# ruanyyyyyyy/point-cloud-process

Hardware: AMD Instinct MI355X
Metric: correspondence-pairs/sec + ms/ICP-iter, 120k-pt KITTI pair (higher is better)
Workload: dtype f64; 1 GPU; point-to-point ICP iteration, 120000 x 120000 KITTI-shaped synthetic scan pair per GPU (BASELINE configs[1]); exact 1-NN via grid; nn=grid, pairs_per_gpu=1, points_src=120000, points_tgt=120000

## Files before the change

point-cloud-process_amd/csrc/pcr_grid_search.hip:

```cpp
#include <atomic>
#include <chrono>
#include <cmath>
#include <cstdlib>
#include <cstring>
#include "pcr_descent.h"
#include "pcr_icp_step.h"

constexpr unsigned int HARD_SCAN_T = 192;
constexpr int HARD_STACK = 160;
constexpr long long ID_NONE = 0x7fffffffffffffffll;
constexpr int H_NLIST = 32;
constexpr int H_CSTRIDE = 32;
__host__ __device__ static inline unsigned int hard_list_cap(long long nq) {
    const long long halves = (nq + 15) / 16;
    return (unsigned int)(((halves + H_NLIST - 1) / H_NLIST) * 16 + 64);
}

template <int G>
__device__ static inline void group_best(double& bd2, long long& bid, unsigned int& bpos) {
#pragma unroll
    for (int off = G / 2; off > 0; off >>= 1) {
        const double od2 = __shfl_xor(bd2, off, 64);
        const long long oid = __shfl_xor(bid, off, 64);
        const unsigned int opos = __shfl_xor(bpos, off, 64);
// ... 649 lines not shown
        const cell_entry en = L->stack[sp];
        const double ecell = gv.cell0 * (double)(1ll << (2 * en.level));
        if (box_dist2(gv, en.level, ecell, en.x, en.y, en.z, ax, ay, az) > bound2) continue;
        const int cl = en.level - 1;
        const unsigned int CX = en.x * 4u + (lane & 3), CY = en.y * 4u + ((lane >> 2) & 3), CZ = en.z * 4u + (lane >> 4);
        const double cdist = box_dist2(gv, cl, ecell * 0.25, CX, CY, CZ, ax, ay, az);
        unsigned int cs = 0, ce = 0;
        const bool cvalid = cdist <= bound2 && lookup_cell(gv.table[cl], gv.mask[cl], CX, CY, CZ, &cs, &ce);
        hard_disperse(gv, L, sp, lane, cvalid, cs, ce, CX, CY, CZ, cl, cdist, ax, ay, az, bd2, bid, bpos, bound2, n_pts, bw);
        ++h_steps;
    }
}

__device__ __forceinline__ static void hard_search(const pcr_grid_view& gv, hard_lds* L, const int lane, const double ax, const double ay, const double az,
                                                   double bound2, bool have_cand, double& bd2, long long& bid, unsigned int& bpos,
                                                   unsigned int& h_steps, unsigned int& h_pts, int& s_level0, double* win = nullptr) {
    double bw[3] = {0.0, 0.0, 0.0};
    const int top = gv.levels - 1;
    bd2 = DBL_MAX;
    bid = ID_NONE;
    bpos = POS_NONE;
    bool clamped = false;
    const int cx = cell_coord(ax, gv.lo[0], gv.inv_cell0, &clamped);
    const int cy = cell_coord(ay, gv.lo[1], gv.inv_cell0, &clamped);
    const int cz = cell_coord(az, gv.lo[2], gv.inv_cell0, &clamped);
    if (!clamped && !have_cand) {
        unsigned int s, e;
        if (lookup_cell(gv.table[0], gv.mask[0], (unsigned int)cx, (unsigned int)cy, (unsigned int)cz, &s, &e)) {
            scan_range(gv.pts, s + lane, e, 64, ax, ay, az, bd2, bid, bpos, bw);
            bound2 = fmin(bound2, wave_min_f64(bd2));
        }
    }
    auto level_for = [&](double b2, int from) {
        double c = gv.cell0 * (double)(1ll << (2 * from));
        for (int l = from; l <= top; ++l) {
            const double safe = c * (1.0 - 1e-9);
            if (safe * safe >= b2) return l;
            c *= 4.0;
        }
        return top + 1;
    };
    have_cand = have_cand || __any(bd2 < DBL_MAX);
    int s_level = clamped ? top + 1 : (have_cand ? level_for(bound2, 0) : 0);
    s_level0 = s_level;
    int sp = 0;
    while (s_level <= top) {
        const int lvl = s_level;
        const double cell = gv.cell0 * (double)(1ll << (2 * lvl));
        bool valid = lane < 27;
        const int X = (cx >> (2 * lvl)) + (lane % 3 - 1), Y = (cy >> (2 * lvl)) + ((lane / 3) % 3 - 1), Z = (cz >> (2 * lvl)) + (lane / 9 - 1);
        const int lim = (int)(PCR_COORD_MAX >> (2 * lvl));
        valid = valid && X >= 0 && Y >= 0 && Z >= 0 && X <= lim && Y <= lim && Z <= lim;
        unsigned int s = 0, e = 0;
        double bdist = 0.0;
        if (valid) {
            bdist = box_dist2(gv, lvl, cell, (unsigned int)X, (unsigned int)Y, (unsigned int)Z, ax, ay, az);
            valid = bdist <= bound2 && lookup_cell(gv.table[lvl], gv.mask[lvl], (unsigned int)X, (unsigned int)Y, (unsigned int)Z, &s, &e);
        }
        hard_disperse(gv, L, sp, lane, valid, s, e, (unsigned int)X, (unsigned int)Y, (unsigned int)Z, lvl, bdist, ax, ay, az, bd2, bid, bpos,
                      bound2, h_pts, bw);
        ++h_steps;
        hard_drain(gv, L, sp, lane, ax, ay, az, bd2, bid, bpos, bound2, h_steps, h_pts, bw);
        const double safe = cell * (1.0 - 1e-9);
        if (safe * safe >= bound2) break;
        s_level = (bound2 < DBL_MAX) ? level_for(bound2, lvl + 1) : lvl + 1;
    }
    if (s_level > top) {
        const double cell = gv.cell0 * (double)(1ll << (2 * top));
        const int b0 = (int)(PCR_COORD_BIAS >> (2 * top));
        bool valid = lane < 8;
        const unsigned int X = b0 + (lane & 1), Y = b0 + ((lane >> 1) & 1), Z = b0 + ((lane >> 2) & 1);
        unsigned int s = 0, e = 0;
        double bdist = 0.0;
        if (valid) {
            bdist = box_dist2(gv, top, cell, X, Y, Z, ax, ay, az);
            valid = bdist <= bound2 && lookup_cell(gv.table[top], gv.mask[top], X, Y, Z, &s, &e);
        }
        hard_disperse(gv, L, sp, lane, valid, s, e, X, Y, Z, top, bdist, ax, ay, az, bd2, bid, bpos, bound2, h_pts, bw);
        ++h_steps;
        hard_drain(gv, L, sp, lane, ax, ay, az, bd2, bid, bpos, bound2, h_steps, h_pts, bw);
    }
    {
        const double m = wave_min_f64(bd2);
        unsigned long long cm = __ballot(bpos != POS_NONE && bd2 == m);
        if (!cm) { bd2 = DBL_MAX; bid = ID_NONE; bpos = POS_NONE; if (win) { win[0] = win[1] = win[2] = 0.0; } return; }
        int wl = (int)__ffsll((long long)cm) - 1;
        cm &= cm - 1;
        if (cm) {
            long long best_id = readlane_i64(bid, wl);
            while (cm) {
                const int l = (int)__ffsll((long long)cm) - 1;
                cm &= cm - 1;
                const long long id_l = readlane_i64(bid, l);
                if (id_l < best_id) { best_id = id_l; wl = l; }
            }
        }
        bd2 = m;
        bid = readlane_i64(bid, wl);
        bpos = (unsigned int)__builtin_amdgcn_readlane((int)bpos, wl);
        if (win) {
#pragma unroll
            for (int k = 0; k < 3; ++k)
                win[k] = readlane_f64(bw[k], wl);
        }
    }
}

__global__ void __launch_bounds__(256)
grid_hard_kernel(pcr_grid_view gv, const work_item* __restrict__ list, const unsigned int* __restrict__ count_p, long long nq, double max_d2, int gated,
                 unsigned int* __restrict__ res_pos, double* __restrict__ res_d2, unsigned long long* __restrict__ dbg,
                 const pcr_icp_dev_state* __restrict__ st) {
    __shared__ hard_lds s_lds[4];
    if (st && st->stop) return;
    const int lane = threadIdx.x & 63, wave = threadIdx.x >> 6;
    hard_lds* L = &s_lds[wave];
    unsigned int l_cnt = lane < H_NLIST ? count_p[H_CSTRIDE * lane] : 0u;
    unsigned int l_inc = l_cnt;
#pragma unroll
    for (int off = 1; off < H_NLIST; off <<= 1) {
        const unsigned int o = __shfl_up(l_inc, off, 64);
        if (lane >= off) l_inc += o;
    }
    const unsigned int count = __shfl(l_inc, H_NLIST - 1, 64);
    const unsigned int l_exc = l_inc - l_cnt;
    const unsigned int l_cap = hard_list_cap(nq);
    for (unsigned int w = blockIdx.x * 4 + wave; w < count; w += gridDim.x * 4) {
        const int hl = (int)__ffsll((long long)__ballot(lane < H_NLIST && l_exc <= w && w < l_exc + l_cnt)) - 1;
        const work_item it = list[(size_t)hl * l_cap + (w - __shfl(l_exc, hl, 64))];
        const unsigned long long h_t0 = dbg ? __builtin_amdgcn_s_memtime() : 0;
        unsigned int h_steps = 0, h_pts = 0;
        int s_level0 = 0;
        double bd2;
        long long bid;
        unsigned int bpos;
        hard_search(gv, L, lane, it.ax, it.ay, it.az, gated ? fmin(it.best_d2, max_d2) : it.best_d2, it.best_pos != POS_NONE, bd2, bid, bpos, h_steps,
                    h_pts, s_level0);
        if (lane == 0) {
            res_pos[it.qi] = bpos;
            if (res_d2) res_d2[it.qi] = bd2;
            if (dbg && w < 60000) {
                dbg[(1 << 17) + w * 4 + 0] = __builtin_amdgcn_s_memtime() - h_t0;
                dbg[(1 << 17) + w * 4 + 1] = ((unsigned long long)h_steps << 32);
                dbg[(1 << 17) + w * 4 + 2] = h_pts;
                dbg[(1 << 17) + w * 4 + 3] = (unsigned long long)(it.best_pos != POS_NONE) | ((unsigned long long)(s_level0 + 1) << 8);
            }
        }
    }
}

constexpr int ACC_SETS = 32;
constexpr int PASS_GROUPS = 32;
constexpr int PASS_SYNC_STRIDE = 32;
constexpr int PASS_SYNC_WORDS = PASS_SYNC_STRIDE * (PASS_GROUPS + 1);
constexpr unsigned long long ITEM_NONE = ~0ull;
constexpr unsigned int POISON_HI = 0xfffffffeu;
__device__ static inline unsigned long long item_poison(unsigned int pass_id) { return ((unsigned long long)POISON_HI << 32) | pass_id; }
#ifndef PCR_PASS_SPIN_LIMIT
#define PCR_PASS_SPIN_LIMIT (1u << 21)
#endif
constexpr unsigned int PASS_SPIN_LIMIT = PCR_PASS_SPIN_LIMIT;
constexpr int Q_BITS = 22;
constexpr unsigned long long Q_MASK = (1ull << Q_BITS) - 1ull;
constexpr long long PASS_MAX_NQ = 1ll << 26;
struct pass_args {
    unsigned long long* items;
    unsigned long long* sync;
    unsigned int cap;
    unsigned long long* acc;
    wt_xyz* prev_xyz;
    double scale, inv_scale;
    pcr_icp_dev_state* st;
    pcr_icp_loop_args la;
    unsigned int* tile_cost;
    unsigned int pass_id;
    unsigned long long* host_block;
    unsigned int notify;
    unsigned int* plog;
};
constexpr int PASS_LOG_WORDS = 3 * PCR_ICP_MAX_LOG + 8;
constexpr size_t HOST_LOG_OFF = (sizeof(pcr_icp_dev_state) + 63) & ~(size_t)63;
constexpr size_t HOST_FLAG_OFF = 8192 - 8;
static_assert(HOST_LOG_OFF + 4 * PASS_LOG_WORDS <= HOST_FLAG_OFF, "state + pass log + flag fit the landing block");
__host__ __device__ static inline unsigned int pass_item_cap(long long nq) {
    const long long tiles = (nq + WT_Q - 1) / WT_Q + 4;
    return (unsigned int)(((tiles + PASS_GROUPS - 1) / PASS_GROUPS) * (WT_Q + 1));
}

__device__ static inline long long to_fixed(double v, double scale) {
    constexpr double BIG = 6755399441055744.0;
    return __double_as_longlong(__builtin_fma(v, scale, BIG)) - __double_as_longlong(BIG);
}

__device__ static inline void acc_fixed_add(unsigned long long* __restrict__ acc, unsigned int set, int lane, double mk, double scale) {
    if (lane < PCR_NMOM - 1 && mk != 0.0)
        atomicAdd(acc + (size_t)(set % ACC_SETS) * PCR_NMOM + lane, (unsigned long long)to_fixed(mk, scale));
}

__device__ static inline void acc_fixed_add_ll(unsigned long long* __restrict__ acc, unsigned int set, int lane, long long v) {
    if (lane < PCR_NMOM - 1 && v != 0) atomicAdd(acc + (size_t)(set % ACC_SETS) * PCR_NMOM + lane, (unsigned long long)v);
}

__device__ static inline unsigned long long ld_dev(const unsigned long long* p) {
    return __hip_atomic_load(p, __ATOMIC_RELAXED, __HIP_MEMORY_SCOPE_AGENT);
}
__device__ static inline void st_dev(unsigned long long* p, unsigned long long v) {
    __hip_atomic_store(p, v, __ATOMIC_RELAXED, __HIP_MEMORY_SCOPE_AGENT);
}

union pass_lds {
    wtile_lds t;
    hard_lds h;
    double xch[WT_Q * (PCR_NMOM - 1)];
    long long xll[WT_Q * (PCR_NMOM - 1)];
};

__device__ __forceinline__ static void pass_serve_item(const pcr_grid_view& gv, pass_lds* L, const int lane, const unsigned long long w, const double max_d2,
                                                       const pass_args& A, unsigned int* __restrict__ res_pos, unsigned long long* __restrict__ dbg,
                                                       const unsigned int dbg_slot, const unsigned long long t_start) {
    const unsigned int w_lo = (unsigned int)w, w_hi = (unsigned int)(w >> 32);
    const double ax = __hiloint2double(__builtin_amdgcn_readlane((int)w_hi, 0), __builtin_amdgcn_readlane((int)w_lo, 0));
    const double ay = __hiloint2double(__builtin_amdgcn_readlane((int)w_hi, 1), __builtin_amdgcn_readlane((int)w_lo, 1));
    const double az = __hiloint2double(__builtin_amdgcn_readlane((int)w_hi, 2), __builtin_amdgcn_readlane((int)w_lo, 2));
    const unsigned int qi = (unsigned int)__builtin_amdgcn_readlane((int)w_lo, 3);
    const float cand_b2 = __uint_as_float((unsigned int)__builtin_amdgcn_readlane((int)w_hi, 3));
    const unsigned long long h_t0 = dbg ? __builtin_amdgcn_s_memtime() : 0;
    unsigned int h_steps = 0, h_pts = 0;
    int s_level0 = 0;
    double bd2;
    long long bid;
    unsigned int bpos;
    const bool have_cand = cand_b2 < INFINITY;
    double win[3];
    hard_search(gv, &L->h, lane, ax, ay, az, have_cand ? fmin((double)cand_b2, max_d2) : max_d2, have_cand, bd2, bid, bpos, h_steps, h_pts, s_level0, win);
    wave_sync();
    if (bpos != POS_NONE) {
        if (lane == 0) {
            pcr_pt b;
            b.x = win[0]; b.y = win[1]; b.z = win[2]; b.id = 0;
            A.prev_xyz[qi] = wt_xyz{b.x, b.y, b.z};
            double m[PCR_NMOM];
#pragma unroll
            for (int k = 0; k < PCR_NMOM; ++k) m[k] = 0.0;
            moments_add(m, gv.origin, ax, ay, az, b, max_d2, 1);
#pragma unroll
            for (int k = 0; k < PCR_NMOM - 1; ++k) L->xch[k] = m[k];
        }
        wave_sync();
        acc_fixed_add(A.acc, qi, lane, lane < PCR_NMOM - 1 ? L->xch[lane] : 0.0, A.scale);
        wave_sync();
    }
    if (lane == 0) {
        res_pos[qi] = bpos;
        if (dbg && dbg_slot < 60000) {
            dbg[(1 << 17) + dbg_slot * 4 + 0] = __builtin_amdgcn_s_memtime() - h_t0;
            dbg[(1 << 17) + dbg_slot * 4 + 1] = ((unsigned long long)h_steps << 32) | (unsigned int)((h_t0 - t_start) >> 4);
            dbg[(1 << 17) + dbg_slot * 4 + 2] = h_pts;
            dbg[(1 << 17) + dbg_slot * 4 + 3] = (unsigned long long)have_cand | ((unsigned long long)(s_level0 + 1) << 8);
        }
    }
}

__device__ __forceinline__ static void pass_finish(const pcr_grid_view& gv, pass_lds* L, const int lane, const pass_args& A, unsigned long long* root,
                                                   unsigned long long* __restrict__ dbg) {
    constexpr int HEAD_WORDS = (int)(pcr::ICP_STATE_HEAD_BYTES / 8);
    static_assert(pcr::ICP_STATE_HEAD_BYTES % 8 == 0 && HEAD_WORDS <= 64, "state head: one word per lane");
    double* const head = L->xch + 32;
    unsigned long long hw = 0, err_w = 0;
    if (lane < HEAD_WORDS) hw = reinterpret_cast<const unsigned long long*>(A.st)[lane];
    if (lane == 63) err_w = ld_dev(root + 16);
    const int mom = lane % PCR_NMOM, part = lane / PCR_NMOM;
    long long sum = 0;
    if (part < 3) {
        constexpr int PER = (ACC_SETS + 2) / 3;
        unsigned long long v[PER];
#pragma unroll
        for (int j = 0; j < PER; ++j) {
            const int set = part + 3 * j;
            v[j] = set < ACC_SETS ? ld_dev(A.acc + (size_t)set * PCR_NMOM + mom) : 0ull;
        }
#pragma unroll
        for (int j = 0; j < PER; ++j) {
            const int set = part + 3 * j;
            if (v[j]) st_dev(A.acc + (size_t)set * PCR_NMOM + mom, 0ull);
            sum += (long long)v[j];
        }
    }
    if (dbg && lane == 0) dbg[(1 << 19) - 4] = __builtin_amdgcn_s_memrealtime();
    sum += __shfl(sum, lane + PCR_NMOM, 64) + __shfl(sum, lane + 2 * PCR_NMOM, 64);
    wave_sync();
    if (dbg && lane == 0) dbg[(1 << 19) - 3] = __builtin_amdgcn_s_memrealtime();
    if (lane < PCR_NMOM) L->xch[lane] = (double)sum * A.inv_scale;
    if (lane < HEAD_WORDS) reinterpret_cast<unsigned long long*>(head)[lane] = hw;
    const bool gave_up = __builtin_amdgcn_readlane((int)(unsigned int)err_w, 63) != 0;
    wave_sync();
    if (lane == 0) {
        pcr_icp_dev_state* hs = reinterpret_cast<pcr_icp_dev_state*>(head);
        if (gave_up) { hs->status = PCR_E_HIP; hs->stop = 1; st_dev(root + 16, 0ull); }
        else pcr::icp_step(hs, L->xch, gv.origin, A.la, A.st->r_diff, A.st->t_diff);
    }
    wave_sync();
    if (dbg && lane == 0) dbg[(1 << 19) - 2] = __builtin_amdgcn_s_memrealtime();
    if (A.plog && lane == 0 && A.pass_id < (unsigned int)PCR_ICP_MAX_LOG) A.plog[A.pass_id] = (unsigned int)__builtin_amdgcn_s_memrealtime();
    if (lane < HEAD_WORDS) reinterpret_cast<unsigned long long*>(A.st)[lane] = reinterpret_cast<const unsigned long long*>(head)[lane];
    if (dbg && lane == 0) dbg[(1 << 19) - 1] = __builtin_amdgcn_s_memrealtime();
    if (A.host_block) {
        const int stop_now = reinterpret_cast<const pcr_icp_dev_state*>(head)->stop;
        if (A.notify || stop_now) {
            asm volatile("s_waitcnt vmcnt(0)" ::: "memory");
            wave_sync();
            constexpr int STATE_WORDS = (int)(sizeof(pcr_icp_dev_state) / 8);
            if (lane < HEAD_WORDS) A.host_block[lane] = reinterpret_cast<const unsigned long long*>(head)[lane];
            for (int w = HEAD_WORDS + lane; w < STATE_WORDS; w += 64) A.host_block[w] = ld_dev(reinterpret_cast<const unsigned long long*>(A.st) + w);
            if (A.plog)
                for (int w = lane; w < PASS_LOG_WORDS / 2; w += 64) A.host_block[HOST_LOG_OFF / 8 + w] = ld_dev(reinterpret_cast<const unsigned long long*>(A.plog) + w);
            __threadfence_system();
            wave_sync();
            if (lane == 0) __hip_atomic_store(A.host_block + HOST_FLAG_OFF / 8, (unsigned long long)A.pass_id + 1ull, __ATOMIC_RELEASE, __HIP_MEMORY_SCOPE_SYSTEM);
        }
    }
}

__device__ __forceinline__ static void tile_set_priority(unsigned int last_cost) {
    const unsigned int lc = (unsigned int)__builtin_amdgcn_readfirstlane((int)last_cost);
    const unsigned int c = lc & 0xffffu, had_open = lc >> 16;
    if (c > 3 * WT_PR) __builtin_amdgcn_s_setprio(3);
    else if (c > 2 * WT_PR) __builtin_amdgcn_s_setprio(2);
    else if (c > WT_PR || had_open) __builtin_amdgcn_s_setprio(1);
}
__device__ __forceinline__ static void tile_record_cost(const wt_state& S, int lane, unsigned int* tile_cost, unsigned int tile) {
    wave_sync();
    __builtin_amdgcn_s_setprio(0);
    const unsigned int n_open = (unsigned int)__popcll(__ballot(S.open && lane < WT_Q));
    if (lane == 0) tile_cost[tile] = (S.staged < 0xffffu ? S.staged : 0xffffu) | (n_open << 16);
}

struct tile_nb {
    pcr_pt b;
    bool proven, known;
};
__device__ __forceinline__ static void tile_neighbour(const pcr_pt* pts, const wt_state& S, const wt_pre& P, int lane, tile_nb& nb) {
    nb.proven = lane < WT_Q && S.won != POS_NONE;
    nb.b.x = nb.b.y = nb.b.z = 0.0; nb.b.id = 0;
    nb.known = nb.proven && S.won == P.seed_pos;
    if (nb.proven && !nb.known) nb.b = as_global(pts)[S.won];
}

__device__ __forceinline__ static unsigned long long publish_reserve(unsigned long long* sync, unsigned long long um, bool unres, int lane, unsigned int g,
                                                            unsigned int n_groups, unsigned int& tg) {
    const unsigned int rank = (unsigned int)__popcll(um & ((1ull << lane) - 1ull));
    tg = (g + rank) % n_groups;
    unsigned long long slot_w = 0;
    if (unres) slot_w = __hip_atomic_fetch_add(sync + (size_t)PASS_SYNC_STRIDE * tg, 1ull, __ATOMIC_RELAXED, __HIP_MEMORY_SCOPE_AGENT);
    return slot_w;
}
template <bool DEV_STORE>
__device__ __forceinline__ static void publish_store(unsigned long long* items, unsigned int cap, unsigned int tg, unsigned long long slot_w, const wt_state& S,
                                            unsigned int id) {
    unsigned long long* it = items + ((size_t)tg * cap + (size_t)(slot_w & Q_MASK)) * 4;
    const bool cand = !S.clamped && S.cand_pos != POS_NONE;
    auto put = [it](int k, unsigned long long v) {
        if (DEV_STORE) st_dev(it + k, v);
        else it[k] = v;
    };
    put(0, S.ax == S.ax ? (unsigned long long)__double_as_longlong(S.ax) : 0x7ff8000000000000ull);
    put(1, S.ay == S.ay ? (unsigned long long)__double_as_longlong(S.ay) : 0x7ff8000000000000ull);
    put(2, S.az == S.az ? (unsigned long long)__double_as_longlong(S.az) : 0x7ff8000000000000ull);
    put(3, (unsigned long long)id | ((unsigned long long)__float_as_uint(cand ? S.bound2 : INFINITY) << 32));
}

__device__ __forceinline__ static void tile_fold_moments(pass_lds* L, int lane, const wt_state& S, const wt_pre& P, tile_nb& nb, const double origin[3], double max_d2,
                                                wt_xyz* prev_xyz, const double& scale, unsigned long long* acc, unsigned int tile) {
    double m[PCR_NMOM];
#pragma unroll
    for (int k = 0; k < PCR_NMOM; ++k) m[k] = 0.0;
    if (nb.proven) {
        if (nb.known) { nb.b.x = P.seed_b.x; nb.b.y = P.seed_b.y; nb.b.z = P.seed_b.z; }
        else prev_xyz[S.qi] = wt_xyz{nb.b.x, nb.b.y, nb.b.z};
        moments_add(m, origin, S.ax, S.ay, S.az, nb.b, max_d2, 1);
    }
    if (lane < WT_Q) {
#pragma unroll
        for (int k = 0; k < PCR_NMOM - 1; ++k) L->xll[lane * (PCR_NMOM - 1) + k] = to_fixed(m[k], scale);
    }
    wave_sync();
    long long tot = 0;
    if (lane < PCR_NMOM - 1) {
#pragma unroll 8
        for (int j = 0; j < WT_Q; ++j) tot += L->xll[j * (PCR_NMOM - 1) + lane];
    }
    acc_fixed_add_ll(acc, tile, lane, tot);
}

struct drain_part {
    unsigned int cnt, exc, total;
};
__device__ __forceinline__ static drain_part drain_partition(const unsigned long long* sync, int lane) {
    static_assert(PASS_GROUPS <= 64, "one group per lane");
    drain_part d;
    d.cnt = lane < PASS_GROUPS ? (unsigned int)(sync[(size_t)PASS_SYNC_STRIDE * lane] & Q_MASK) : 0u;
    d.exc = wave_excl_scan_u32(d.cnt, lane, &d.total);
    return d;
}
__device__ __forceinline__ static unsigned long long drain_take(const drain_part& d, unsigned long long* items, unsigned int cap, unsigned int w_i, int lane) {
    const int grp = (int)__ffsll((long long)__ballot(((lane < PASS_GROUPS) & (d.exc <= w_i)) && w_i < d.exc + d.cnt)) - 1;
    const unsigned int idx = w_i - (unsigned int)__builtin_amdgcn_readlane((int)d.exc, grp);
    unsigned long long* it = items + ((size_t)grp * cap + idx) * 4;
    unsigned long long w = ITEM_NONE;
    if (lane < 4) {
        w = it[lane];
        it[lane] = ITEM_NONE;
    }
    return w;
}

#ifndef PCR_PASS_DIAG
#define PCR_PASS_DIAG 0
#endif
__global__ void __launch_bounds__(256) __attribute__((amdgpu_waves_per_eu(PCR_WT_WAVES, 8)))
grid_pass_kernel(const pcr_grid_view* __restrict__ gvp, pcr_grid_view gv, pcr_pt* __restrict__ q, long long nq, double max_d2, int xcd_remap,
                 unsigned int pcap_arg, unsigned int pcap_busy, unsigned int* __restrict__ res_pos, unsigned long long* __restrict__ dbg_arg, int use_prev, int inline_queue,
                 pass_args A) {
    unsigned long long* const dbg = PCR_PASS_DIAG ? dbg_arg : nullptr;
    __shared__ pass_lds s_lds[4];
    const int lane = threadIdx.x & 63, wave = __builtin_amdgcn_readfirstlane((int)(threadIdx.x >> 6));
    const unsigned int tile = wtile_block(xcd_remap) * 4 + wave;
    wt_pre P;
    wtile_preload(tile, lane, q, nq, res_pos, use_prev ? A.prev_xyz : nullptr, P);
    const unsigned int last_cost = use_prev ? A.tile_cost[tile] : 0u;
    unsigned int pcap = pcap_arg;
    if (pcap_busy > pcap_arg && A.plog) {
        const unsigned int prev_items = A.pass_id > 0 && A.pass_id <= (unsigned int)PCR_ICP_MAX_LOG ? A.plog[2 * PCR_ICP_MAX_LOG + A.pass_id - 1] : 0xffffffffu;
        if ((unsigned long long)prev_items * 16ull > (unsigned long long)nq) pcap = pcap_busy;
        pcap = (unsigned int)__builtin_amdgcn_readfirstlane((int)pcap);
    }
    const pcr_xform x = A.st->x;
    if (A.st->stop) return;
    tile_set_priority(last_cost);
    const unsigned long long t_start = dbg ? __builtin_amdgcn_s_memtime() : 0;
    const unsigned long long rt_start = dbg ? __builtin_amdgcn_s_memrealtime() : 0;
    unsigned long long rt_tile = 0, rt_acc = 0;
    unsigned int n_items = 0, n_polls = 0, n_casfail = 0;
    pass_lds* L = &s_lds[wave];
    const unsigned int n_waves = gridDim.x * 4;
    const unsigned int g = tile % PASS_GROUPS;
    const unsigned int g_tiles = n_waves / PASS_GROUPS + (g < n_waves % PASS_GROUPS ? 1u : 0u);
    unsigned long long* const g_q = A.sync + (size_t)PASS_SYNC_STRIDE * g;
    unsigned long long* const g_started = g_q + 16;
    unsigned long long* const g_ticket = g_q + 17;
    unsigned long long* const items = A.items + (size_t)g * A.cap * 4;
    if (lane == 0) __hip_atomic_fetch_add(g_started, 1ull, __ATOMIC_RELAXED, __HIP_MEMORY_SCOPE_AGENT);
    const unsigned int n_groups = n_waves < (unsigned int)PASS_GROUPS ? n_waves : (unsigned int)PASS_GROUPS;
    wt_state S;
    wtile_search(*gvp, &L->t, tile, lane, P, q, nq, x, 1, 1, max_d2, 1, pcap, res_pos, nullptr, dbg, use_prev ? A.prev_xyz : nullptr, S, inline_queue ? A.sync + 16 : nullptr,
                 (unsigned int)PASS_SYNC_STRIDE, n_groups, n_waves);
    tile_record_cost(S, lane, A.tile_cost, tile);
    if (dbg) rt_tile = __builtin_amdgcn_s_memrealtime();
    tile_nb nb;
    tile_neighbour(gv.pts, S, P, lane, nb);
    bool all_started = false;
    if (inline_queue) {
        all_started = S.probe != 0;
        if (!all_started) {
            unsigned long long sv = 0;
            if (lane < (int)n_groups) sv = ld_dev(A.sync + (size_t)PASS_SYNC_STRIDE * lane + 16);
            const bool ok = lane < (int)n_groups && (unsigned int)sv == n_waves / PASS_GROUPS + ((unsigned int)lane < n_waves % PASS_GROUPS ? 1u : 0u);
            all_started = __ballot(ok) == (n_groups >= 64 ? ~0ull : (1ull << n_groups) - 1ull);
        }
    }
    const bool unres = S.open && lane < WT_Q;
    const unsigned long long um = __ballot(unres);
    unsigned int mine = 0;
    bool have_claim = false;
    unsigned long long own = 0;
    unsigned long long* const root = A.sync + (size_t)PASS_SYNC_STRIDE * PASS_GROUPS;
    {
        unsigned int tg;
        const unsigned long long slot_w = publish_reserve(A.sync, um, unres, lane, g, n_groups, tg);
        asm volatile("" :: "v"(slot_w) : "memory");
        if (lane == 0)
            own = __hip_atomic_fetch_add(g_q, (1ull << (2 * Q_BITS)) | (all_started ? 1ull << Q_BITS : 0ull), __ATOMIC_RELAXED, __HIP_MEMORY_SCOPE_AGENT);
        if (unres) publish_store<true>(A.items, A.cap, tg, slot_w, S, (unsigned int)S.qi);
    }
    tile_fold_moments(L, lane, S, P, nb, gv.origin, max_d2, A.prev_xyz, A.scale, A.acc, tile);
    wave_sync();
    {
        {
            const unsigned int o_lo = (unsigned int)__builtin_amdgcn_readfirstlane((int)(unsigned int)own), o_hi = (unsigned int)__builtin_amdgcn_readfirstlane((int)(unsigned int)(own >> 32));
            own = ((unsigned long long)o_hi << 32) | o_lo;
        }
        if (all_started) {
            have_claim = true;
            mine = (unsigned int)((own >> Q_BITS) & Q_MASK);
        }
        if ((unsigned int)(own >> (2 * Q_BITS)) == g_tiles - 1u && inline_queue) {
            int fin = 0;
            if (lane == 0) fin = __hip_atomic_fetch_add(root + 8, 1ull, __ATOMIC_RELAXED, __HIP_MEMORY_SCOPE_AGENT) == (unsigned long long)(n_groups - 1u) ? 1 : 0;
            if (__builtin_amdgcn_readfirstlane(fin)) {
                if (lane == 0) st_dev(root + 8, 0ull);
                unsigned long long qw = 0;
                if (lane < (int)n_groups) qw = ld_dev(A.sync + (size_t)PASS_SYNC_STRIDE * lane);
                const unsigned int R_l = (unsigned int)(qw & Q_MASK);
                for (unsigned int gg = 0; gg < n_groups; ++gg) {
                    const unsigned int R = (unsigned int)__builtin_amdgcn_readlane((int)R_l, (int)gg);
                    const unsigned int gt = n_waves / PASS_GROUPS + (gg < n_waves % PASS_GROUPS ? 1u : 0u);
                    unsigned long long* const base_g = A.items + (size_t)gg * A.cap * 4;
                    for (unsigned int k = lane; k < gt; k += 64) st_dev(base_g + (size_t)(R + k) * 4 + 3, item_poison(A.pass_id));
                }
            }
        }
    }
    if (dbg) rt_acc = __builtin_amdgcn_s_memrealtime();
    if (dbg && lane == 0) {
        atomicAdd(&dbg[blockIdx.x * 4 + 1], S.dbg_pairs);
        atomicAdd(&dbg[blockIdx.x * 4 + 2], (unsigned long long)S.dbg_passes);
        atomicAdd(&dbg[blockIdx.x * 4 + 3], (unsigned long long)__popcll(um));
        atomicMax(&dbg[blockIdx.x * 4 + 0], __builtin_amdgcn_s_memtime() - t_start);
    }
    if (!inline_queue) return;
    bool failed = false, left_by_poison = false;
    for (;;) {
        if (!have_claim) {
            if (!all_started) {
                unsigned long long sv = 0;
                if (lane < (int)n_groups) sv = ld_dev(A.sync + (size_t)PASS_SYNC_STRIDE * lane + 16);
                const bool ok = lane < (int)n_groups && (unsigned int)sv == n_waves / PASS_GROUPS + ((unsigned int)lane < n_waves % PASS_GROUPS ? 1u : 0u);
                all_started = __ballot(ok) == (n_groups >= 64 ? ~0ull : (1ull << n_groups) - 1ull);
            }
            if (all_started) {
                unsigned long long old = 0;
                if (lane == 0) old = __hip_atomic_fetch_add(g_q, 1ull << Q_BITS, __ATOMIC_RELAXED, __HIP_MEMORY_SCOPE_AGENT);
                const unsigned int o_lo = (unsigned int)__builtin_amdgcn_readfirstlane((int)(unsigned int)old), o_hi = (unsigned int)__builtin_amdgcn_readfirstlane((int)(unsigned int)(old >> 32));
                old = ((unsigned long long)o_hi << 32) | o_lo;
                mine = (unsigned int)((old >> Q_BITS) & Q_MASK);
            } else {
                unsigned long long qw = 0;
                if (lane == 0) qw = ld_dev(g_q);
                const unsigned int q_lo = (unsigned int)__builtin_amdgcn_readfirstlane((int)(unsigned int)qw), q_hi = (unsigned int)__builtin_amdgcn_readfirstlane((int)(unsigned int)(qw >> 32));
                qw = ((unsigned long long)q_hi << 32) | q_lo;
                mine = (unsigned int)((qw >> Q_BITS) & Q_MASK);
                if (mine >= (unsigned int)(qw & Q_MASK)) break;
                int got = 0;
                if (lane == 0) {
                    unsigned long long expect = qw;
                    got = __hip_atomic_compare_exchange_strong(g_q, &expect, qw + (1ull << Q_BITS), __ATOMIC_RELAXED, __ATOMIC_RELAXED, __HIP_MEMORY_SCOPE_AGENT) ? 1 : 0;
                }
                if (!__builtin_amdgcn_readfirstlane(got)) { ++n_casfail; continue; }
            }
        }
        have_claim = false;
        unsigned long long* it = items + (size_t)mine * 4;
        unsigned long long w = ITEM_NONE;
        bool poisoned = false;
        for (unsigned int spins = 0;; ++spins) {
            if (lane < 4) w = ld_dev(it + lane);
            const unsigned int w3_lo = (unsigned int)__builtin_amdgcn_readlane((int)(unsigned int)w, 3), w3_hi = (unsigned int)__builtin_amdgcn_readlane((int)(unsigned int)(w >> 32), 3);
            poisoned = w3_hi == POISON_HI && w3_lo == A.pass_id;
            const unsigned long long mk = __ballot(lane < 4 && w != ITEM_NONE && !(lane == 3 && w3_hi == POISON_HI));
            if (poisoned || mk == 0xfull) break;
            if (spins >= PASS_SPIN_LIMIT) { failed = true; break; }
            ++n_polls;
            __builtin_amdgcn_s_sleep(16);
        }
        if (failed) break;
        if (poisoned) { left_by_poison = true; break; }
        if (lane < 4) st_dev(it + lane, ITEM_NONE);
        ++n_items;
        pass_serve_item(gv, L, lane, w, max_d2, A, res_pos, dbg, g + PASS_GROUPS * mine, t_start);
    }
    const unsigned long long rt_loop = dbg ? __builtin_amdgcn_s_memrealtime() : 0;
    asm volatile("s_waitcnt vmcnt(0)" ::: "memory");
    int last = 0;
    {
        if (lane == 0) {
            const unsigned long long tg_old = __hip_atomic_fetch_add(g_ticket, 1ull | (left_by_poison ? 1ull << 32 : 0ull) | (failed ? 1ull << 48 : 0ull), __ATOMIC_RELAXED,
                                                                     __HIP_MEMORY_SCOPE_AGENT);
            if ((unsigned int)tg_old == g_tiles - 1u) {
                const bool g_clean = ((tg_old >> 32) & 0xffffull) != 0 || left_by_poison;
                const bool g_failed = (tg_old >> 48) != 0 || failed;
                const unsigned long long tr_old = __hip_atomic_fetch_add(root, 1ull | (g_clean ? 1ull << 32 : 0ull) | (g_failed ? 1ull << 48 : 0ull), __ATOMIC_RELAXED,
                                                                         __HIP_MEMORY_SCOPE_AGENT);
                if ((unsigned int)tr_old == n_groups - 1u) {
                    last = ((unsigned int)((tr_old >> 32) & 0xffffull) + (g_clean ? 1u : 0u) == n_groups) ? 1 : 2;
                    if ((tr_old >> 48) != 0 || g_failed) last = 3;
                }
            }
        }
    }
    if (dbg && lane == 0) {
        unsigned long long* d = dbg + (1 << 19) + (size_t)(blockIdx.x * 4 + wave) * 8;
        d[0] = rt_start; d[1] = rt_tile; d[2] = rt_acc; d[3] = rt_loop; d[4] = n_items; d[5] = n_polls | ((unsigned long long)n_casfail << 32); d[6] = S.dbg_pairs | ((unsigned long long)S.dbg_passes << 40) | ((unsigned long long)__popcll(um) << 48); d[7] = __builtin_amdgcn_s_memrealtime();
    }
    last = __builtin_amdgcn_readfirstlane(last);
    if (!last) return;
    if (last == 3 && dbg_arg && lane == 0) atomicAdd(&dbg_arg[(1 << 19) - 16], 1ull);
    if (last >= 2) {
        unsigned long long qw = 0;
        if (lane < (int)n_groups) qw = ld_dev(A.sync + (size_t)PASS_SYNC_STRIDE * lane);
        const unsigned int r_l = (unsigned int)(qw & Q_MASK);
        const unsigned int c_l = last == 3 ? 0u : (unsigned int)((qw >> Q_BITS) & Q_MASK);
        unsigned long long left = __ballot(lane < (int)n_groups && c_l < r_l);
        while (left) {
            const int gg = (int)__ffsll((long long)left) - 1;
            left &= left - 1;
            const unsigned int c0 = (unsigned int)__builtin_amdgcn_readlane((int)c_l, gg), r0 = (unsigned int)__builtin_amdgcn_readlane((int)r_l, gg);
            for (unsigned int i = c0; i < r0; ++i) {
                unsigned long long* it = A.items + ((size_t)gg * A.cap + i) * 4;
                unsigned long long w = ITEM_NONE;
                bool arrived = false;
                const unsigned int patience = last == 3 ? 64u : (PASS_SPIN_LIMIT < (1u << 21) ? (1u << 21) : PASS_SPIN_LIMIT);
                bool served_before = false;
                for (unsigned int spins = 0; spins < patience; ++spins) {
                    if (lane < 4) w = ld_dev(it + lane);
                    const unsigned int w3_hi = (unsigned int)__builtin_amdgcn_readlane((int)(unsigned int)(w >> 32), 3);
                    if (__ballot(lane < 4 && w != ITEM_NONE && !(lane == 3 && w3_hi == POISON_HI)) == 0xfull) { arrived = true; break; }
                    if (last == 3 && __ballot(lane < 4 && w == ITEM_NONE) == 0xfull) { served_before = true; break; }
                    __builtin_amdgcn_s_sleep(2);
                }
                if (served_before) continue;
                if (lane < 4) st_dev(it + lane, ITEM_NONE);
                if (!arrived) { if (lane == 0) st_dev(root + 16, 1ull); continue; }
                pass_serve_item(gv, L, lane, w, max_d2, A, res_pos, dbg, 59999u, t_start);
            }
        }
        asm volatile("s_waitcnt vmcnt(0)" ::: "memory");
    }
    if (lane < (int)n_groups) {
        st_dev(A.sync + (size_t)PASS_SYNC_STRIDE * lane, 0ull);
        st_dev(A.sync + (size_t)PASS_SYNC_STRIDE * lane + 16, 0ull);
        st_dev(A.sync + (size_t)PASS_SYNC_STRIDE * lane + 17, 0ull);
    }
    if (lane == 0) st_dev(root, 0ull);
    pass_finish(gv, L, lane, A, root, dbg);
}

__global__ void __launch_bounds__(256) __attribute__((amdgpu_waves_per_eu(PCR_WT_WAVES, 8)))
grid_drain_kernel(pcr_grid_view gv, double max_d2, unsigned int* __restrict__ res_pos, unsigned long long* __restrict__ dbg, pass_args A) {
    __shared__ pass_lds s_lds[4];
    if (A.st->stop) return;
    const unsigned long long t_start = dbg ? __builtin_amdgcn_s_memtime() : 0;
    const unsigned long long t_rt_start = __builtin_amdgcn_s_memrealtime();
    const int lane = threadIdx.x & 63, wave = threadIdx.x >> 6;
    pass_lds* L = &s_lds[wave];
    const drain_part dp = drain_partition(A.sync, lane);
    const unsigned int total = dp.total;
    const unsigned int n_waves = gridDim.x * 4;
    if (dbg && blockIdx.x == 0 && threadIdx.x == 0) dbg[(1 << 19) - 8] = total;
    if (A.plog && blockIdx.x == 0 && threadIdx.x == 0 && A.pass_id < (unsigned int)PCR_ICP_MAX_LOG) {
        A.plog[PCR_ICP_MAX_LOG + A.pass_id] = (unsigned int)t_rt_start | 1u;
        A.plog[2 * PCR_ICP_MAX_LOG + A.pass_id] = total;
    }
    for (unsigned int w_i = blockIdx.x * 4 + wave; w_i < total; w_i += n_waves)
        pass_serve_item(gv, L, lane, drain_take(dp, A.items, A.cap, w_i, lane), max_d2, A, res_pos, dbg, w_i, t_start);
    asm volatile("s_waitcnt vmcnt(0)" ::: "memory");
    unsigned long long* const root = A.sync + (size_t)PASS_SYNC_STRIDE * PASS_GROUPS;
    const unsigned int wid = blockIdx.x * 4 + wave;
    const unsigned int n_groups = n_waves < (unsigned int)PASS_GROUPS ? n_waves : (unsigned int)PASS_GROUPS;
    const unsigned int g = wid % n_groups;
    const unsigned int g_size = n_waves / n_groups + (g < n_waves % n_groups ? 1u : 0u);
    unsigned long long* const g_ticket = A.sync + (size_t)PASS_SYNC_STRIDE * g + 17;
    int last = 0;
    if (lane == 0) {
        if (__hip_atomic_fetch_add(g_ticket, 1ull, __ATOMIC_RELAXED, __HIP_MEMORY_SCOPE_AGENT) == (unsigned long long)(g_size - 1u)) {
            st_dev(g_ticket, 0ull);
            if (__hip_atomic_fetch_add(root, 1ull, __ATOMIC_RELAXED, __HIP_MEMORY_SCOPE_AGENT) == (unsigned long long)(n_groups - 1u)) {
                st_dev(root, 0ull);
                last = 1;
            }
        }
    }
    if (!__builtin_amdgcn_readfirstlane(last)) return;
    if (lane < PASS_GROUPS) {
        st_dev(A.sync + (size_t)PASS_SYNC_STRIDE * lane, 0ull);
        st_dev(A.sync + (size_t)PASS_SYNC_STRIDE * lane + 16, 0ull);
    }
    pass_finish(gv, L, lane, A, root, dbg);
}

__global__ void grid_finalize_nn1_kernel(pcr_grid_view gv, const pcr_pt* __restrict__ q, long long nq, const unsigned int* __restrict__ res_pos,
                                         const double* __restrict__ res_d2, double max_d2, int gated, int* __restrict__ idx_out,
                                         double* __restrict__ d2_out, unsigned int* __restrict__ hard_count) {
    const long long qi = (long long)blockIdx.x * blockDim.x + threadIdx.x;
    if (qi < H_NLIST) hard_count[H_CSTRIDE * qi] = 0;
    if (qi >= nq) return;
    const unsigned int pos = res_pos[qi];
    const double d2 = res_d2[qi];
    const long long qid = q[qi].id;
    int id = -1;
    if (pos != POS_NONE && (!gated || d2 < max_d2)) id = (int)gv.pts[pos].id;
    idx_out[qid] = id;
    d2_out[qid] = (pos == POS_NONE) ? INFINITY : d2;
}

__global__ void __launch_bounds__(256)
grid_accumulate_kernel(pcr_grid_view gv, const pcr_pt* __restrict__ q, long long nq, pcr_xform x, int apply_x,
                       const unsigned int* __restrict__ res_pos, double max_d2, int gated, double* __restrict__ partials,
                       unsigned int* __restrict__ ticket, double* __restrict__ out, unsigned int* __restrict__ hard_count,
                       pcr_icp_dev_state* __restrict__ st, pcr_icp_loop_args la, wt_xyz* __restrict__ prev_xyz) {
    __shared__ double s_part[4][PCR_NMOM];
    if (st && st->stop) return;
    double m[PCR_NMOM];
#pragma unroll
    for (int k = 0; k < PCR_NMOM; ++k) m[k] = 0.0;
    const long long stride = (long long)gridDim.x * blockDim.x;
    for (long long q0 = (long long)blockIdx.x * blockDim.x + threadIdx.x; q0 < nq; q0 += 4 * stride) {
        unsigned int pos[4];
        pcr_pt p[4], b[4];
#pragma unroll
        for (int u = 0; u < 4; ++u) {
            const long long qi = q0 + u * stride;
            pos[u] = qi < nq ? res_pos[qi] : POS_NONE;
        }
#pragma unroll
        for (int u = 0; u < 4; ++u) {
            const long long qi = q0 + u * stride;
            if (qi < nq) p[u] = q[qi];
        }
#pragma unroll
        for (int u = 0; u < 4; ++u)
            if (pos[u] != POS_NONE) b[u] = gv.pts[pos[u]];
        if (prev_xyz) {
#pragma unroll
            for (int u = 0; u < 4; ++u)
                if (pos[u] != POS_NONE) prev_xyz[q0 + u * stride] = wt_xyz{b[u].x, b[u].y, b[u].z};
        }
#pragma unroll
        for (int u = 0; u < 4; ++u) {
            if (pos[u] == POS_NONE) continue;
            double ax = p[u].x, ay = p[u].y, az = p[u].z;
            if (apply_x) xform_apply(x, p[u], &ax, &ay, &az);
            const double d2 = dist2(ax, ay, az, b[u]);
            if (gated && !(d2 < max_d2)) continue;
            const double a0 = ax - gv.origin[0], a1 = ay - gv.origin[1], a2 = az - gv.origin[2];
            const double b0 = b[u].x - gv.origin[0], b1 = b[u].y - gv.origin[1], b2 = b[u].z - gv.origin[2];
            m[0] += 1.0;
            m[1] += a0; m[2] += a1; m[3] += a2;
            m[4] += b0; m[5] += b1; m[6] += b2;
            m[7] += b0 * a0; m[8] += b0 * a1; m[9] += b0 * a2;
            m[10] += b1 * a0; m[11] += b1 * a1; m[12] += b1 * a2;
            m[13] += b2 * a0; m[14] += b2 * a1; m[15] += b2 * a2;
            m[16] += (a0 * a0 + a1 * a1) + a2 * a2;
            m[17] += (b0 * b0 + b1 * b1) + b2 * b2;
            m[18] += d2;
        }
    }
#pragma unroll
    for (int k = 0; k < PCR_NMOM - 1; ++k) m[k] = wave_total_f64(m[k]);
    const int wave = threadIdx.x >> 6, lane = threadIdx.x & 63;
    if (lane == 63) {
#pragma unroll
        for (int k = 0; k < PCR_NMOM; ++k) s_part[wave][k] = m[k];
    }
    __syncthreads();
    if (threadIdx.x < PCR_NMOM) {
        const double v = (s_part[0][threadIdx.x] + s_part[1][threadIdx.x]) + (s_part[2][threadIdx.x] + s_part[3][threadIdx.x]);
        partials[(long long)blockIdx.x * PCR_NMOM + threadIdx.x] = v;
    }
    if (ticket == nullptr) {
        if (blockIdx.x == 0 && threadIdx.x < H_NLIST) hard_count[H_CSTRIDE * threadIdx.x] = 0;
        return;
    }
    __shared__ unsigned int s_last;
    asm volatile("s_waitcnt vmcnt(0)" ::: "memory");
    __syncthreads();
    if (threadIdx.x == 0) {
        __builtin_amdgcn_fence(__ATOMIC_RELEASE, "agent");
        asm volatile("s_waitcnt vmcnt(0)" ::: "memory");
        const unsigned int t = __hip_atomic_fetch_add(ticket, 1u, __ATOMIC_RELAXED, __HIP_MEMORY_SCOPE_AGENT);
        s_last = (t == gridDim.x - 1) ? 1u : 0u;
        if (s_last) {
            __builtin_amdgcn_fence(__ATOMIC_ACQUIRE, "agent");
            asm volatile("s_waitcnt vmcnt(0)" ::: "memory");
            *ticket = 0;
        }
    }
    __syncthreads();
    if (!s_last) return;
    if (threadIdx.x < H_NLIST) hard_count[H_CSTRIDE * threadIdx.x] = 0;
    __shared__ double s_red[8][32];
    const int k = threadIdx.x & 31, slice = threadIdx.x >> 5;
    double v = 0.0;
    if (k < PCR_NMOM) {
        for (int b0 = slice; b0 < (int)gridDim.x; b0 += 64) {
            double t[8];
#pragma unroll
            for (int u = 0; u < 8; ++u) {
// ... 463 lines not shown
```

Before: 3.367 billion correspondences/s.

## Let closer wave finish pass early via per-group landed counters

Adds a per-group 'landed' counter that records when each tile's published items and each served item have completed their writes. The wave that closes the inline queue polls these counters and, once every group shows all tiles landed and all items served, runs the pass finish immediately instead of waiting for the last ticket holder. The aim is to shorten the tail synchronisation of the fused grid pass. It adds extra atomics and polling and a more intricate termination protocol, with a closed flag in the ticket words and a separate cleanup path.

```diff
diff --git a/point-cloud-process_amd/csrc/pcr_grid_search.hip b/point-cloud-process_amd/csrc/pcr_grid_search.hip
--- a/point-cloud-process_amd/csrc/pcr_grid_search.hip
+++ b/point-cloud-process_amd/csrc/pcr_grid_search.hip
@@ -825,6 +825,8 @@
 constexpr int PASS_GROUPS = 32;
 constexpr int PASS_SYNC_STRIDE = 32;
 constexpr int PASS_SYNC_WORDS = PASS_SYNC_STRIDE * (PASS_GROUPS + 1);
+constexpr int PASS_LANDED = 18;
+constexpr unsigned int PASS_CLAIM_PATIENCE = 64;
 constexpr unsigned long long ITEM_NONE = ~0ull;
 constexpr unsigned int POISON_HI = 0xfffffffeu;
 __device__ static inline unsigned long long item_poison(unsigned int pass_id) { return ((unsigned long long)POISON_HI << 32) | pass_id; }
@@ -1086,6 +1088,33 @@
     return w;
 }
 
+__device__ __forceinline__ static unsigned long long pass_ticket_group(unsigned long long* g_ticket, bool left_by_poison, bool failed, bool closing) {
+    return __hip_atomic_fetch_add(g_ticket, 1ull | (left_by_poison ? 1ull << 32 : 0ull) | (failed ? 1ull << 48 : 0ull) | (closing ? 1ull << 63 : 0ull), __ATOMIC_RELAXED,
+                                  __HIP_MEMORY_SCOPE_AGENT);
+}
+__device__ __forceinline__ static int pass_ticket_root(unsigned long long tg_old, unsigned long long* root, unsigned int g_tiles, unsigned int n_groups, bool left_by_poison,
+                                                       bool failed, bool closing) {
+    if ((unsigned int)tg_old != g_tiles - 1u) return 0;
+    const bool g_clean = ((tg_old >> 32) & 0xffffull) != 0 || left_by_poison;
+    const bool g_failed = ((tg_old >> 48) & 0x7fffull) != 0 || failed;
+    const bool g_closed = (tg_old >> 63) != 0 || closing;
+    const unsigned long long tr_old = __hip_atomic_fetch_add(root, 1ull | (g_clean ? 1ull << 32 : 0ull) | (g_failed ? 1ull << 48 : 0ull) | (g_closed ? 1ull << 63 : 0ull),
+                                                             __ATOMIC_RELAXED, __HIP_MEMORY_SCOPE_AGENT);
+    if ((unsigned int)tr_old != n_groups - 1u) return 0;
+    int last = ((unsigned int)((tr_old >> 32) & 0xffffull) + (g_clean ? 1u : 0u) == n_groups) ? 1 : 2;
+    if (((tr_old >> 48) & 0x7fffull) != 0 || g_failed) last = 3;
+    return last | (((tr_old >> 63) != 0 || g_closed) ? 4 : 0);
+}
+__device__ __forceinline__ static void pass_clean_sync(unsigned long long* sync, unsigned long long* root, unsigned int n_groups, int lane) {
+    if (lane < (int)n_groups) {
+        st_dev(sync + (size_t)PASS_SYNC_STRIDE * lane, 0ull);
+        st_dev(sync + (size_t)PASS_SYNC_STRIDE * lane + 16, 0ull);
+        st_dev(sync + (size_t)PASS_SYNC_STRIDE * lane + 17, 0ull);
+        st_dev(sync + (size_t)PASS_SYNC_STRIDE * lane + PASS_LANDED, 0ull);
+    }
+    if (lane == 0) st_dev(root, 0ull);
+}
+
 #ifndef PCR_PASS_DIAG
 #define PCR_PASS_DIAG 0
 #endif
@@ -1120,6 +1149,7 @@
     unsigned long long* const g_q = A.sync + (size_t)PASS_SYNC_STRIDE * g;
     unsigned long long* const g_started = g_q + 16;
     unsigned long long* const g_ticket = g_q + 17;
+    unsigned long long* const g_landed = g_q + PASS_LANDED;
     unsigned long long* const items = A.items + (size_t)g * A.cap * 4;
     if (lane == 0) __hip_atomic_fetch_add(g_started, 1ull, __ATOMIC_RELAXED, __HIP_MEMORY_SCOPE_AGENT);
     const unsigned int n_groups = n_waves < (unsigned int)PASS_GROUPS ? n_waves : (unsigned int)PASS_GROUPS;
@@ -1144,6 +1174,14 @@
     const unsigned long long um = __ballot(unres);
     unsigned int mine = 0;
     bool have_claim = false;
+    bool tile_pending = inline_queue != 0;
+    auto tile_landed = [&]() {
+        tile_pending = false;
+        asm volatile("s_waitcnt vmcnt(0)" ::: "memory");
+        if (lane == 0) __hip_atomic_fetch_add(g_q + PASS_LANDED, 1ull << 32, __ATOMIC_RELAXED, __HIP_MEMORY_SCOPE_AGENT);
+    };
+    bool closer = false, c_complete = false;
+    unsigned int R_own = 0;
     unsigned long long own = 0;
     unsigned long long* const root = A.sync + (size_t)PASS_SYNC_STRIDE * PASS_GROUPS;
     {
@@ -1169,10 +1207,19 @@
             int fin = 0;
             if (lane == 0) fin = __hip_atomic_fetch_add(root + 8, 1ull, __ATOMIC_RELAXED, __HIP_MEMORY_SCOPE_AGENT) == (unsigned long long)(n_groups - 1u) ? 1 : 0;
             if (__builtin_amdgcn_readfirstlane(fin)) {
+                closer = true;
+                tile_landed();
                 if (lane == 0) st_dev(root + 8, 0ull);
-                unsigned long long qw = 0;
-                if (lane < (int)n_groups) qw = ld_dev(A.sync + (size_t)PASS_SYNC_STRIDE * lane);
+                unsigned long long qw = 0, lw = 0;
+                if (lane < (int)n_groups) {
+                    qw = ld_dev(A.sync + (size_t)PASS_SYNC_STRIDE * lane);
+                    lw = ld_dev(A.sync + (size_t)PASS_SYNC_STRIDE * lane + PASS_LANDED);
+                }
                 const unsigned int R_l = (unsigned int)(qw & Q_MASK);
+                const unsigned int gt_l = n_waves / PASS_GROUPS + ((unsigned int)lane < n_waves % PASS_GROUPS ? 1u : 0u);
+                c_complete = __ballot(lane < (int)n_groups && lw == (((unsigned long long)gt_l << 32) | R_l)) == (n_groups >= 64 ? ~0ull : (1ull << n_groups) - 1ull);
+                R_own = (unsigned int)__builtin_amdgcn_readlane((int)R_l, (int)g);
+                if (dbg && lane == 0) dbg[(1 << 19) - 6] = __builtin_amdgcn_s_memrealtime();
                 for (unsigned int gg = 0; gg < n_groups; ++gg) {
                     const unsigned int R = (unsigned int)__builtin_amdgcn_readlane((int)R_l, (int)gg);
                     const unsigned int gt = n_waves / PASS_GROUPS + (gg < n_waves % PASS_GROUPS ? 1u : 0u);
@@ -1190,7 +1237,7 @@
         atomicMax(&dbg[blockIdx.x * 4 + 0], __builtin_amdgcn_s_memtime() - t_start);
     }
     if (!inline_queue) return;
-    bool failed = false, left_by_poison = false;
+    bool failed = false, left_by_poison = false, served = false;
     for (;;) {
         if (!have_claim) {
             if (!all_started) {
@@ -1205,7 +1252,13 @@
                 const unsigned int o_lo = (unsigned int)__builtin_amdgcn_readfirstlane((int)(unsigned int)old), o_hi = (unsigned int)__builtin_amdgcn_readfirstlane((int)(unsigned int)(old >> 32));
                 old = ((unsigned long long)o_hi << 32) | o_lo;
                 mine = (unsigned int)((old >> Q_BITS) & Q_MASK);
-            } else {
+            }
+            if (served) {
+                served = false;
+                asm volatile("s_waitcnt vmcnt(0)" ::: "memory");
+                if (lane == 0) __hip_atomic_fetch_add(g_landed, 1ull, __ATOMIC_RELAXED, __HIP_MEMORY_SCOPE_AGENT);
+            }
+            if (!all_started) {
                 unsigned long long qw = 0;
                 if (lane == 0) qw = ld_dev(g_q);
                 const unsigned int q_lo = (unsigned int)__builtin_amdgcn_readfirstlane((int)(unsigned int)qw), q_hi = (unsigned int)__builtin_amdgcn_readfirstlane((int)(unsigned int)(qw >> 32));
@@ -1221,6 +1274,7 @@
             }
         }
         have_claim = false;
+        if (closer && mine >= R_own) { left_by_poison = true; break; }
         unsigned long long* it = items + (size_t)mine * 4;
         unsigned long long w = ITEM_NONE;
         bool poisoned = false;
@@ -1228,6 +1282,7 @@
             if (lane < 4) w = ld_dev(it + lane);
             const unsigned int w3_lo = (unsigned int)__builtin_amdgcn_readlane((int)(unsigned int)w, 3), w3_hi = (unsigned int)__builtin_amdgcn_readlane((int)(unsigned int)(w >> 32), 3);
             poisoned = w3_hi == POISON_HI && w3_lo == A.pass_id;
+            if (tile_pending) tile_landed();
             const unsigned long long mk = __ballot(lane < 4 && w != ITEM_NONE && !(lane == 3 && w3_hi == POISON_HI));
             if (poisoned || mk == 0xfull) break;
             if (spins >= PASS_SPIN_LIMIT) { failed = true; break; }
@@ -1239,71 +1294,97 @@
         if (lane < 4) st_dev(it + lane, ITEM_NONE);
         ++n_items;
         pass_serve_item(gv, L, lane, w, max_d2, A, res_pos, dbg, g + PASS_GROUPS * mine, t_start);
+        served = true;
     }
     const unsigned long long rt_loop = dbg ? __builtin_amdgcn_s_memrealtime() : 0;
-    asm volatile("s_waitcnt vmcnt(0)" ::: "memory");
-    int last = 0;
-    {
-        if (lane == 0) {
-            const unsigned long long tg_old = __hip_atomic_fetch_add(g_ticket, 1ull | (left_by_poison ? 1ull << 32 : 0ull) | (failed ? 1ull << 48 : 0ull), __ATOMIC_RELAXED,
-                                                                     __HIP_MEMORY_SCOPE_AGENT);
-            if ((unsigned int)tg_old == g_tiles - 1u) {
-                const bool g_clean = ((tg_old >> 32) & 0xffffull) != 0 || left_by_poison;
-                const bool g_failed = (tg_old >> 48) != 0 || failed;
-                const unsigned long long tr_old = __hip_atomic_fetch_add(root, 1ull | (g_clean ? 1ull << 32 : 0ull) | (g_failed ? 1ull << 48 : 0ull), __ATOMIC_RELAXED,
-                                                                         __HIP_MEMORY_SCOPE_AGENT);
-                if ((unsigned int)tr_old == n_groups - 1u) {
-                    last = ((unsigned int)((tr_old >> 32) & 0xffffull) + (g_clean ? 1u : 0u) == n_groups) ? 1 : 2;
-                    if ((tr_old >> 48) != 0 || g_failed) last = 3;
-                }
-            }
-        }
-    }
-    if (dbg && lane == 0) {
+    auto stamp_wave = [&]() {
         unsigned long long* d = dbg + (1 << 19) + (size_t)(blockIdx.x * 4 + wave) * 8;
         d[0] = rt_start; d[1] = rt_tile; d[2] = rt_acc; d[3] = rt_loop; d[4] = n_items; d[5] = n_polls | ((unsigned long long)n_casfail << 32); d[6] = S.dbg_pairs | ((unsigned long long)S.dbg_passes << 40) | ((unsigned long long)__popcll(um) << 48); d[7] = __builtin_amdgcn_s_memrealtime();
-    }
-    last = __builtin_amdgcn_readfirstlane(last);
-    if (!last) return;
-    if (last == 3 && dbg_arg && lane == 0) atomicAdd(&dbg_arg[(1 << 19) - 16], 1ull);
-    if (last >= 2) {
-        unsigned long long qw = 0;
-        if (lane < (int)n_groups) qw = ld_dev(A.sync + (size_t)PASS_SYNC_STRIDE * lane);
-        const unsigned int r_l = (unsigned int)(qw & Q_MASK);
-        const unsigned int c_l = last == 3 ? 0u : (unsigned int)((qw >> Q_BITS) & Q_MASK);
-        unsigned long long left = __ballot(lane < (int)n_groups && c_l < r_l);
-        while (left) {
-            const int gg = (int)__ffsll((long long)left) - 1;
-            left &= left - 1;
-            const unsigned int c0 = (unsigned int)__builtin_amdgcn_readlane((int)c_l, gg), r0 = (unsigned int)__builtin_amdgcn_readlane((int)r_l, gg);
-            for (unsigned int i = c0; i < r0; ++i) {
-                unsigned long long* it = A.items + ((size_t)gg * A.cap + i) * 4;
-                unsigned long long w = ITEM_NONE;
-                bool arrived = false;
-                const unsigned int patience = last == 3 ? 64u : (PASS_SPIN_LIMIT < (1u << 21) ? (1u << 21) : PASS_SPIN_LIMIT);
-                bool served_before = false;
-                for (unsigned int spins = 0; spins < patience; ++spins) {
-                    if (lane < 4) w = ld_dev(it + lane);
-                    const unsigned int w3_hi = (unsigned int)__builtin_amdgcn_readlane((int)(unsigned int)(w >> 32), 3);
-                    if (__ballot(lane < 4 && w != ITEM_NONE && !(lane == 3 && w3_hi == POISON_HI)) == 0xfull) { arrived = true; break; }
-                    if (last == 3 && __ballot(lane < 4 && w == ITEM_NONE) == 0xfull) { served_before = true; break; }
-                    __builtin_amdgcn_s_sleep(2);
+    };
+    if (tile_pending) {
+        tile_landed();
+        asm volatile("s_waitcnt vmcnt(0)" ::: "memory");
+    }
+    bool complete = false;
+    if (closer && !failed) {
+        complete = c_complete;
+        if (!complete) {
+            const unsigned int gt_l = n_waves / PASS_GROUPS + ((unsigned int)lane < n_waves % PASS_GROUPS ? 1u : 0u);
+            const unsigned long long full = n_groups >= 64 ? ~0ull : (1ull << n_groups) - 1ull;
+            for (unsigned int polls = 1;; ++polls) {
+                unsigned long long qw = 0, lw = 0;
+                if (lane < (int)n_groups) {
+                    qw = ld_dev(A.sync + (size_t)PASS_SYNC_STRIDE * lane);
+                    lw = ld_dev(A.sync + (size_t)PASS_SYNC_STRIDE * lane + PASS_LANDED);
                 }
-                if (served_before) continue;
-                if (lane < 4) st_dev(it + lane, ITEM_NONE);
-                if (!arrived) { if (lane == 0) st_dev(root + 16, 1ull); continue; }
-                pass_serve_item(gv, L, lane, w, max_d2, A, res_pos, dbg, 59999u, t_start);
-            }
-        }
-        asm volatile("s_waitcnt vmcnt(0)" ::: "memory");
-    }
-    if (lane < (int)n_groups) {
-        st_dev(A.sync + (size_t)PASS_SYNC_STRIDE * lane, 0ull);
-        st_dev(A.sync + (size_t)PASS_SYNC_STRIDE * lane + 16, 0ull);
-        st_dev(A.sync + (size_t)PASS_SYNC_STRIDE * lane + 17, 0ull);
-    }
-    if (lane == 0) st_dev(root, 0ull);
+                const unsigned int r_l = (unsigned int)(qw & Q_MASK), c_l = (unsigned int)((qw >> Q_BITS) & Q_MASK);
+                if (__ballot(lane < (int)n_groups && lw == (((unsigned long long)gt_l << 32) | r_l)) == full) { complete = true; break; }
+                if (polls >= PASS_SPIN_LIMIT) break;
+                if (polls >= PASS_CLAIM_PATIENCE && __ballot(lane < (int)n_groups && c_l < r_l) != 0ull) break;
+                __builtin_amdgcn_s_sleep(2);
+            }
+        }
+        if (complete) {
+            if (dbg && lane == 0) dbg[(1 << 19) - 5] = __builtin_amdgcn_s_memrealtime();
+            if (dbg_arg && lane == 0) atomicAdd(&dbg_arg[(1 << 19) - 15], 1ull);
+        }
+    }
+    asm volatile("s_waitcnt vmcnt(0)" ::: "memory");
+    unsigned long long tg_old = 0;
+    if (lane == 0) tg_old = pass_ticket_group(g_ticket, left_by_poison, failed, complete);
+    if (!complete) {
+        int last = 0;
+        if (lane == 0) last = pass_ticket_root(tg_old, root, g_tiles, n_groups, left_by_poison, failed, false);
+        if (dbg && lane == 0) stamp_wave();
+        last = __builtin_amdgcn_readfirstlane(last);
+        if (!last) return;
+        if ((last & 3) == 3 && dbg_arg && lane == 0) atomicAdd(&dbg_arg[(1 << 19) - 16], 1ull);
+        if (last & 4) {
+            pass_clean_sync(A.sync, root, n_groups, lane);
+            return;
+        }
+        if (last >= 2) {
+            unsigned long long qw = 0;
+            if (lane < (int)n_groups) qw = ld_dev(A.sync + (size_t)PASS_SYNC_STRIDE * lane);
+            const unsigned int r_l = (unsigned int)(qw & Q_MASK);
+            const unsigned int c_l = last == 3 ? 0u : (unsigned int)((qw >> Q_BITS) & Q_MASK);
+            unsigned long long left = __ballot(lane < (int)n_groups && c_l < r_l);
+            while (left) {
+                const int gg = (int)__ffsll((long long)left) - 1;
+                left &= left - 1;
+                const unsigned int c0 = (unsigned int)__builtin_amdgcn_readlane((int)c_l, gg), r0 = (unsigned int)__builtin_amdgcn_readlane((int)r_l, gg);
+                for (unsigned int i = c0; i < r0; ++i) {
+                    unsigned long long* it = A.items + ((size_t)gg * A.cap + i) * 4;
+                    unsigned long long w = ITEM_NONE;
+                    bool arrived = false;
+                    const unsigned int patience = last == 3 ? 64u : (PASS_SPIN_LIMIT < (1u << 21) ? (1u << 21) : PASS_SPIN_LIMIT);
+                    bool served_before = false;
+                    for (unsigned int spins = 0; spins < patience; ++spins) {
+                        if (lane < 4) w = ld_dev(it + lane);
+                        const unsigned int w3_hi = (unsigned int)__builtin_amdgcn_readlane((int)(unsigned int)(w >> 32), 3);
+                        if (__ballot(lane < 4 && w != ITEM_NONE && !(lane == 3 && w3_hi == POISON_HI)) == 0xfull) { arrived = true; break; }
+                        if (last == 3 && __ballot(lane < 4 && w == ITEM_NONE) == 0xfull) { served_before = true; break; }
+                        __builtin_amdgcn_s_sleep(2);
+                    }
+                    if (served_before) continue;
+                    if (lane < 4) st_dev(it + lane, ITEM_NONE);
+                    if (!arrived) { if (lane == 0) st_dev(root + 16, 1ull); continue; }
+                    pass_serve_item(gv, L, lane, w, max_d2, A, res_pos, dbg, 59999u, t_start);
+                }
+            }
+            asm volatile("s_waitcnt vmcnt(0)" ::: "memory");
+        }
+        pass_clean_sync(A.sync, root, n_groups, lane);
+    }
     pass_finish(gv, L, lane, A, root, dbg);
+    if (!complete) return;
+    int last_c = 0;
+    if (lane == 0) last_c = pass_ticket_root(tg_old, root, g_tiles, n_groups, left_by_poison, false, true);
+    if (dbg && lane == 0) stamp_wave();
+    last_c = __builtin_amdgcn_readfirstlane(last_c);
+    if (!last_c) return;
+    if ((last_c & 3) == 3 && dbg_arg && lane == 0) atomicAdd(&dbg_arg[(1 << 19) - 16], 1ull);
+    pass_clean_sync(A.sync, root, n_groups, lane);
 }
 
 __global__ void __launch_bounds__(256) __attribute__((amdgpu_waves_per_eu(PCR_WT_WAVES, 8)))
```

Result: no change. 3.364 billion correspondences/s (-0.1%).
